# DIAGNijmegen/bodyct-dram-emph-subtype

Hardware: AMD Instinct MI355X
Metric: CT volumes/sec (train step, 1x128x256x256) (higher is better)
Workload: dtype f32; 1 GPU; BASELINE configs[1]: resnet18segcls train step (fwd+loss+bwd+Adam), batch 2/GPU, 1x128x256x256, fp32, inputs resident in HBM; global_batch=2, parallelism=dp1, hip_graph=False, streams=2

## Files before the change

### bodyct-dram-emph-subtype_amd/csrc/stem.hip

```cpp
#include "common.h"

namespace {

constexpr int PZ = 13, PY = 21, PX = 21;
constexpr int PATCH = PZ * PY * PX;
constexpr int PXP = 24;
constexpr int PATCHP = PZ * PY * PXP;
constexpr int WLP = 96;
constexpr int KT = 50;
constexpr int WPT = (KT * 64 + 255) / 256;

struct StemGeom {
  int B, D, H, W, Do, Ho, Wo;
  int nz, ny, nx, tiles_per_b, nblk;
};

template <typename T>
__global__ __launch_bounds__(256, 2) void stem_fwd_kernel(const float* __restrict__ x,
                                                          const float* __restrict__ w,
                                                          T* __restrict__ y, float* __restrict__ stats,
                                                          const StemGeom g) {
  __shared__ __attribute__((aligned(16))) float lds[PATCHP + KT * WLP];
  float* patch = lds;
  float* wl = lds + PATCHP;
  const int tid = threadIdx.x, lane = tid & 63, wave = tid >> 6;
  const int li = lane & 31, lh = lane >> 5;

  int L = xcd_remap(blockIdx.x, g.nblk);
  const int b = L / g.tiles_per_b;
  int r = L - b * g.tiles_per_b;
  const int txi = r % g.nx; r /= g.nx;
  const int tyi = r % g.ny;
  const int tzi = r / g.ny;
  const int z0 = tzi * 4, y0 = tyi * 8, x0 = txi * 8;

  for (int idx = tid; idx < PATCH; idx += 256) {
    const int pz = idx / (PY * PX);
    const int rem = idx - pz * (PY * PX);
    const int py = rem / PX, px = rem - py * PX;
    const int zi = 2 * z0 - 3 + pz, yi = 2 * y0 - 3 + py, xi = 2 * x0 - 3 + px;
    const bool ok = (zi >= 0) & (zi < g.D) & (yi >= 0) & (yi < g.H) & (xi >= 0) & (xi < g.W);
    patch[(pz * PY + py) * PXP + px] = ok ? x[(((long)b * g.D + zi) * g.H + yi) * g.W + xi] : 0.f;
  }

  float rw[WPT];
  auto load_w = [&](int kz) {
#pragma unroll
    for (int p = 0; p < WPT; ++p) {
      const int idx = p * 256 + tid;
      const int t = idx >> 6, co = idx & 63;
      rw[p] = (idx < KT * 64 && t < 49) ? w[co * 343 + kz * 49 + t] : 0.f;
    }
  };
  auto store_w = [&]() {
#pragma unroll
    for (int p = 0; p < WPT; ++p) {
      const int idx = p * 256 + tid;
      if (idx < KT * 64) wl[(idx >> 6) * WLP + (idx & 63)] = rw[p];
    }
  };

  f32x16 acc[2][2];
#pragma unroll
  for (int mi = 0; mi < 2; ++mi)
#pragma unroll
    for (int nj = 0; nj < 2; ++nj)
#pragma unroll
      for (int e = 0; e < 16; ++e) acc[mi][nj][e] = 0.f;

  int abase[2];
#pragma unroll
  for (int mi = 0; mi < 2; ++mi) abase[mi] = (2 * wave) * (PY * PXP) + (2 * (4 * mi + (li >> 3))) * PXP + 2 * (li & 7);

  load_w(0);
  for (int kz = 0; kz < 7; ++kz) {
    __syncthreads();
    store_w();
    __syncthreads();
    if (kz + 1 < 7) load_w(kz + 1);
    const float* pk = patch + kz * (PY * PXP);
#pragma unroll
    for (int kk = 0; kk < KT / 2; ++kk) {
      constexpr int dummy = 0;
      (void)dummy;
      const int k0 = 2 * kk, k1 = 2 * kk + 1;
      const int o0 = (k0 < 49) ? (k0 / 7) * PXP + (k0 % 7) : 0;
      const int o1 = (k1 < 49) ? (k1 / 7) * PXP + (k1 % 7) : 0;
      const int ko = lh ? o1 : o0;
      const float a0 = pk[abase[0] + ko];
      const float a1 = pk[abase[1] + ko];
      const float b0 = wl[(2 * kk + lh) * WLP + li];
      const float b1 = wl[(2 * kk + lh) * WLP + 32 + li];
      acc[0][0] = __builtin_amdgcn_mfma_f32_32x32x2f32(a0, b0, acc[0][0], 0, 0, 0);
      acc[0][1] = __builtin_amdgcn_mfma_f32_32x32x2f32(a0, b1, acc[0][1], 0, 0, 0);
      acc[1][0] = __builtin_amdgcn_mfma_f32_32x32x2f32(a1, b0, acc[1][0], 0, 0, 0);
      acc[1][1] = __builtin_amdgcn_mfma_f32_32x32x2f32(a1, b1, acc[1][1], 0, 0, 0);
    }
  }

  float s1[2] = {0.f, 0.f}, s2[2] = {0.f, 0.f};
#pragma unroll
  for (int mi = 0; mi < 2; ++mi) {
#pragma unroll
    for (int e = 0; e < 16; ++e) {
      const int row = wave * 64 + mi * 32 + (e & 3) + 8 * (e >> 2) + 4 * lh;
      const int zo = z0 + (row >> 6), yo = y0 + ((row >> 3) & 7), xo = x0 + (row & 7);
      if ((zo < g.Do) & (yo < g.Ho) & (xo < g.Wo)) {
        const long o = ((((long)b * g.Do + zo) * g.Ho + yo) * g.Wo + xo) * 64 + li;
#pragma unroll
        for (int nj = 0; nj < 2; ++nj) {
          const float v = acc[mi][nj][e];
          st1<T>(y, o + nj * 32, v);
          s1[nj] += v;
          s2[nj] += v * v;
        }
      }
    }
  }
  if (stats) {
    __syncthreads();
    float* red = lds;
#pragma unroll
    for (int nj = 0; nj < 2; ++nj) {
      const float t1 = s1[nj] + __shfl_xor(s1[nj], 32, 64);
      const float t2 = s2[nj] + __shfl_xor(s2[nj], 32, 64);
      if (lh == 0) {
        red[(wave * 2 + 0) * 64 + nj * 32 + li] = t1;
        red[(wave * 2 + 1) * 64 + nj * 32 + li] = t2;
      }
    }
    __syncthreads();
    if (tid < 128) {
      const int which = tid >> 6, c = tid & 63;
      const float v = red[(0 + which) * 64 + c] + red[(2 + which) * 64 + c] + red[(4 + which) * 64 + c] +
                      red[(6 + which) * 64 + c];
      stats[((long)L * 2 + which) * 64 + c] = v;
    }
  }
}

constexpr int GZ = 7, GY = 21, GX = 21;
constexpr int GPATCH = GZ * GY * GX;
constexpr int GXP = 27;
constexpr int GPATCHP = GZ * GY * GXP;
constexpr int NTAP = 352;
constexpr int GLDY = 96;
constexpr int GPT = (GPATCH + 255) / 256;

struct StemWGeom {
  int B, D, H, W, Do, Ho, Wo;
  int ny, nx;
  int total;
};

template <typename T>
__global__ __launch_bounds__(256, 2) void stem_wgrad_kernel(const float* __restrict__ x,
                                                            const T* __restrict__ dy,
                                                            float* __restrict__ slab, const StemWGeom g) {
  __shared__ __attribute__((aligned(16))) float lds[GPATCHP + 3 + 64 * GLDY];
  float* patch = lds;
  float* dyl = lds + GPATCHP + 3;
  const int tid = threadIdx.x, lane = tid & 63, wave = tid >> 6;
  const int li = lane & 31, lh = lane >> 5;
  const int ntw = (wave < 3) ? 3 : 2;

  int toff[3];
#pragma unroll
  for (int j = 0; j < 3; ++j) {
    const int tap = 32 * (wave + 4 * j) + li;
    const int kz = tap / 49, rem = tap - kz * 49, ky = rem / 7, kx = rem - ky * 7;
    toff[j] = (tap < 343 ? kz * (GY * GXP) + ky * GXP + kx : 0) + 2 * lh;
  }

  f32x16 acc[3][2];
#pragma unroll
  for (int j = 0; j < 3; ++j)
#pragma unroll
    for (int mi = 0; mi < 2; ++mi)
#pragma unroll
      for (int e = 0; e < 16; ++e) acc[j][mi][e] = 0.f;

  float rp[GPT];
  float4 rd[4];
  auto load_tile = [&](int st) {
    int r = st;
    const int txi = r % g.nx; r /= g.nx;
    const int tyi = r % g.ny; r /= g.ny;
    const int zo = r % g.Do;
    const int b = r / g.Do;
    const int y0 = tyi * 8, x0 = txi * 8;
#pragma unroll
    for (int p = 0; p < GPT; ++p) {
      const int idx = p * 256 + tid;
      const int pz = idx / (GY * GX);
      const int rem = idx - pz * (GY * GX);
      const int py = rem / GX, px = rem - py * GX;
      const int zi = 2 * zo - 3 + pz, yi = 2 * y0 - 3 + py, xi = 2 * x0 - 3 + px;
      const bool ok = (idx < GPATCH) & (zi >= 0) & (zi < g.D) & (yi >= 0) & (yi < g.H) & (xi >= 0) & (xi < g.W);
      rp[p] = ok ? x[(((long)b * g.D + zi) * g.H + yi) * g.W + xi] : 0.f;
    }
#pragma unroll
    for (int p = 0; p < 4; ++p) {
      const int idx = p * 256 + tid;
      const int v = idx >> 4, c4 = idx & 15;
      const int yo = y0 + (v >> 3), xo = x0 + (v & 7);
      const bool ok = (yo < g.Ho) & (xo < g.Wo);
      const long o = ((((long)b * g.Do + zo) * g.Ho + yo) * g.Wo + xo) * 64 + c4 * 4;
      rd[p] = ok ? ld4<T>(dy, o) : make_float4(0.f, 0.f, 0.f, 0.f);
    }
  };
  auto store_tile = [&]() {
#pragma unroll
    for (int p = 0; p < GPT; ++p) {
      const int idx = p * 256 + tid;
      if (idx < GPATCH) {
        const int pz = idx / (GY * GX), rem = idx - pz * (GY * GX);
        patch[(pz * GY + rem / GX) * GXP + rem % GX] = rp[p];
      }
    }
#pragma unroll
    for (int p = 0; p < 4; ++p) {
      const int idx = p * 256 + tid;
      *reinterpret_cast<float4*>(&dyl[(idx >> 4) * GLDY + (idx & 15) * 4]) = rd[p];
    }
  };

  int st = blockIdx.x;
  if (st < g.total) load_tile(st);
  for (; st < g.total; st += gridDim.x) {
    __syncthreads();
    store_tile();
    __syncthreads();
    if (st + (int)gridDim.x < g.total) load_tile(st + gridDim.x);
#pragma unroll 8
    for (int kk = 0; kk < 32; ++kk) {
      const int vbase = (2 * (kk >> 2)) * GXP + 4 * (kk & 3);
      const float a0 = dyl[(2 * kk + lh) * GLDY + li];
      const float a1 = dyl[(2 * kk + lh) * GLDY + 32 + li];
#pragma unroll
      for (int j = 0; j < 3; ++j) {
        if (j < ntw) {
          const float bv = patch[vbase + toff[j]];
          acc[j][0] = __builtin_amdgcn_mfma_f32_32x32x2f32(a0, bv, acc[j][0], 0, 0, 0);
          acc[j][1] = __builtin_amdgcn_mfma_f32_32x32x2f32(a1, bv, acc[j][1], 0, 0, 0);
        }
      }
    }
  }
  float* sl = slab + (long)blockIdx.x * 64 * NTAP;
#pragma unroll
  for (int j = 0; j < 3; ++j) {
    if (j < ntw) {
#pragma unroll
      for (int mi = 0; mi < 2; ++mi)
#pragma unroll
        for (int e = 0; e < 16; ++e) {
          const int co = 32 * mi + (e & 3) + 8 * (e >> 2) + 4 * lh;
          sl[co * NTAP + 32 * (wave + 4 * j) + li] = acc[j][mi][e];
        }
    }
  }
}

__global__ __launch_bounds__(256) void stem_wgrad_reduce_kernel(const float* __restrict__ slab, float* __restrict__ dw,
                                                                int nslab) {
  __shared__ float part[4][64];
  const int r = threadIdx.x & 63, kg = threadIdx.x >> 6;
  const int i = blockIdx.x * 64 + r;
  const bool live = i < 64 * NTAP;
  float p[8];
// ... 9 lines not shown
  }
  part[kg][r] = ((p[0] + p[1]) + (p[2] + p[3])) + ((p[4] + p[5]) + (p[6] + p[7]));
  __syncthreads();
  if (kg == 0 && live) {
    const int co = i / NTAP, tap = i - co * NTAP;
    if (tap < 343) dw[co * 343 + tap] = (part[0][r] + part[1][r]) + (part[2][r] + part[3][r]);
  }
}

inline int stem_out(int n) { return (n + 6 - 7) / 2 + 1; }
inline int stem_wgrad_blocks(int total) { return total < 512 ? total : 512; }

}

extern "C" int dram_stem_num_tiles(int B, int Do, int Ho, int Wo) {
  return B * ((Do + 3) / 4) * ((Ho + 7) / 8) * ((Wo + 7) / 8);
}

template <typename T>
static int stem_fwd_impl(const float* x, const float* w, T* y, float* stats_partial, int B, int D, int H, int W,
                         dram_stream_t stream) {
  if (!x || !w || !y || B < 1 || D < 1 || H < 1 || W < 1) return DRAM_ERR_BAD_ARG;
  StemGeom g{};
  g.B = B; g.D = D; g.H = H; g.W = W;
  g.Do = stem_out(D); g.Ho = stem_out(H); g.Wo = stem_out(W);
  if ((long long)B * g.Do * g.Ho * g.Wo * 64 >= (1LL << 31)) return DRAM_ERR_UNSUPPORTED;
  g.nz = (g.Do + 3) / 4; g.ny = (g.Ho + 7) / 8; g.nx = (g.Wo + 7) / 8;
  g.tiles_per_b = g.nz * g.ny * g.nx;
  g.nblk = B * g.tiles_per_b;
  const double vo = (double)B * g.Do * g.Ho * g.Wo;
  DramProf prof(DRAM_FAM_STEM, 0, 2.0 * vo * 64.0 * 343.0,
                4.0 * ((double)B * D * H * W + 64.0 * 343.0) + sizeof(T) * vo * 64.0, (hipStream_t)stream);
  hipLaunchKernelGGL((stem_fwd_kernel<T>), dim3(g.nblk), dim3(256), 0, (hipStream_t)stream, x, w, y, stats_partial, g);
  DRAM_LAUNCH_CHECK();
  return DRAM_OK;
}
extern "C" int dram_stem_fwd(const float* x, const float* w, float* y, float* stats_partial, int B, int D,
                             int H, int W, dram_stream_t stream) {
  return stem_fwd_impl<float>(x, w, y, stats_partial, B, D, H, W, stream);
}
extern "C" int dram_stem_fwd_bf16(const float* x, const float* w, void* y, float* stats_partial, int B, int D,
                                  int H, int W, dram_stream_t stream) {
  return stem_fwd_impl<bf16_t>(x, w, (bf16_t*)y, stats_partial, B, D, H, W, stream);
}

extern "C" size_t dram_stem_bwd_weight_workspace(int B, int D, int H, int W) {
  const int Do = stem_out(D), Ho = stem_out(H), Wo = stem_out(W);
  const int total = B * Do * ((Ho + 7) / 8) * ((Wo + 7) / 8);
  return (size_t)stem_wgrad_blocks(total) * 64 * NTAP * sizeof(float);
}

template <typename T>
static int stem_bwd_weight_impl(const float* x, const T* dy, float* dw, int B, int D, int H, int W, void* workspace,
                                size_t workspace_bytes, dram_stream_t stream) {
  if (!x || !dy || !dw || B < 1 || D < 1 || H < 1 || W < 1) return DRAM_ERR_BAD_ARG;
  StemWGeom g{};
  g.B = B; g.D = D; g.H = H; g.W = W;
  g.Do = stem_out(D); g.Ho = stem_out(H); g.Wo = stem_out(W);
  g.ny = (g.Ho + 7) / 8; g.nx = (g.Wo + 7) / 8;
  g.total = B * g.Do * g.ny * g.nx;
  const int nblk = stem_wgrad_blocks(g.total);
  if (!workspace || workspace_bytes < (size_t)nblk * 64 * NTAP * sizeof(float)) return DRAM_ERR_WORKSPACE;
  hipStream_t s = (hipStream_t)stream;
  const double vo = (double)B * g.Do * g.Ho * g.Wo;
  DramProf prof(DRAM_FAM_STEM, 1, 2.0 * vo * 64.0 * 343.0,
                4.0 * ((double)B * D * H * W + 64.0 * 343.0) + sizeof(T) * vo * 64.0, s);
  hipLaunchKernelGGL((stem_wgrad_kernel<T>), dim3(nblk), dim3(256), 0, s, x, dy, (float*)workspace, g);
  DRAM_LAUNCH_CHECK();
  hipLaunchKernelGGL(stem_wgrad_reduce_kernel, dim3((64 * NTAP + 63) / 64), dim3(256), 0, s,
                     (const float*)workspace, dw, nblk);
  DRAM_LAUNCH_CHECK();
  return DRAM_OK;
}
extern "C" int dram_stem_bwd_weight(const float* x, const float* dy, float* dw, int B, int D, int H, int W,
                                    void* workspace, size_t workspace_bytes, dram_stream_t stream) {
  return stem_bwd_weight_impl<float>(x, dy, dw, B, D, H, W, workspace, workspace_bytes, stream);
}
extern "C" int dram_stem_bwd_weight_bf16(const float* x, const void* dy, float* dw, int B, int D, int H, int W,
                                         void* workspace, size_t workspace_bytes, dram_stream_t stream) {
  return stem_bwd_weight_impl<bf16_t>(x, (const bf16_t*)dy, dw, B, D, H, W, workspace, workspace_bytes, stream);
}
```

### bodyct-dram-emph-subtype_amd/engine.py

```python
from __future__ import annotations

import os
import time
from typing import Dict, List, Optional

import torch

from . import ops
from .ops import ConvGeom

Tensor = torch.Tensor

ARCHS = {
    "resnet18": ("basic", (2, 2, 2, 2)),
    "resnet34": ("basic", (3, 4, 6, 3)),
    "resnet50": ("bottleneck", (3, 4, 6, 3)),
}
EXPANSION = {"basic": 1, "bottleneck": 4}
STAGES = ((64, 1, 1), (128, 2, 1), (256, 1, 2), (512, 1, 4))
BN_EPS = 1e-5
BN_MOMENTUM = 0.1


class _State:
# ... 36 lines not shown

    def _bn_fwd(self, st: _State, y: Tensor, sp: Optional[Tensor], bnp: str, residual, rs, relu=True, pool=False,
                apply=True):
        P = st.P
        count = float(y.numel() // y.shape[-1])
        count_dev = None
        if st.training:
            if st.dist is not None and st.dist.sync_bn:
                flat, sums = ops.reduce_partials(sp, tail=count)
                st.dist.all_reduce_stats(flat)
                count_dev = flat[-1:]
                mean, invstd, scale, shift = ops.bn_finalize(sums, count, P[bnp + ".weight"], P[bnp + ".bias"],
                                                             P[bnp + ".running_mean"], P[bnp + ".running_var"],
                                                             BN_MOMENTUM, BN_EPS, True, count_dev)
            else:
                mean, invstd, scale, shift = ops.bn_fold_finalize(sp, count, P[bnp + ".weight"], P[bnp + ".bias"],
                                                                  P[bnp + ".running_mean"], P[bnp + ".running_var"],
                                                                  BN_MOMENTUM, BN_EPS)
            st.nbt.append(P[bnp + ".num_batches_tracked"])
        else:
            mean, invstd, scale, shift = ops.bn_finalize(None, 1.0, P[bnp + ".weight"], P[bnp + ".bias"],
                                                         P[bnp + ".running_mean"], P[bnp + ".running_var"],
                                                         BN_MOMENTUM, BN_EPS, False)
            if st.need_grad:
                st.eval_ss[bnp] = (scale, shift)
        if not apply:
            z = None
        elif pool:
            z = ops.bn_maxpool_fwd(y, scale, shift)
        else:
            z = ops.bn_apply(y, scale, shift, residual, rs, relu)
        return z, mean, invstd, (count, count_dev), (None if residual is not None else (scale, shift))

    def _bn_bwd_eval(self, st: _State, c: dict, dz: Tensor) -> Tensor:
        bnp = c["bn"]
        scale, shift = st.eval_ss[bnp]
        zmask = c["z"] if c.get("ss") is None else None
        if st.dist is not None:
            self._flush_wgrad(st)
        if st.need_param:
            part = ops.bn_bwd_reduce(dz, zmask, c["y"], c["mean"], c["invstd"], True, scale, shift)
            _, sf = ops.reduce_partials(part, want_f32=True)
            st.grads[bnp + ".weight"] = sf[1]
            st.grads[bnp + ".bias"] = sf[0]
        y = c["y"] if zmask is None else None
        if c.get("b") and st.need_param:
            dy, colpart = ops.bn_bwd_apply_eval(dz, zmask, y, scale, shift, True, want_colsum=True)
            if colpart is None:
                colpart = ops.colsum(dy)
            st.grads[c["b"]] = ops.reduce_partials(colpart)[0].float()
            return dy
        return ops.bn_bwd_apply_eval(dz, zmask, y, scale, shift, True)

    def _bn_bwd(self, st: _State, c: dict, dz: Tensor) -> Tensor:
        if not st.training:
            return self._bn_bwd_eval(st, c, dz)
        bnp = c["bn"]
        zmask, (sc, sh) = (c["z"], (None, None)) if c.get("ss") is None else (None, c["ss"])
        part = c.pop("part", None)
        if part is None:
            part = ops.bn_bwd_reduce(dz, zmask, c["y"], c["mean"], c["invstd"], True, sc, sh)
        sums, sf = ops.reduce_partials(part, want_f32=True)
        st.grads[bnp + ".weight"] = sf[1]
        st.grads[bnp + ".bias"] = sf[0]
        count, count_dev = c["count"]
        if st.dist is not None and st.dist.sync_bn:
            work = st.dist.all_reduce_stats_async(sums)
            self._flush_wgrad(st)
            work.wait()
        if c.get("b"):
            dy, colpart = ops.bn_bwd_apply(dz, zmask, c["y"], c["mean"], c["invstd"], st.P[bnp + ".weight"], sums,
                                           count, True, sc, sh, want_colsum=True, count_dev=count_dev)
            if colpart is None:
                colpart = ops.colsum(dy)
            st.grads[c["b"]] = ops.reduce_partials(colpart)[0].float()
            return dy
        return ops.bn_bwd_apply(dz, zmask, c["y"], c["mean"], c["invstd"], st.P[bnp + ".weight"], sums, count,
                                True, sc, sh, count_dev=count_dev)

    def _conv_bn_fwd(self, st: _State, x, wname: str, bname: Optional[str], bnp: str, k: int, stride: int,
                     pad: int, dil: int, residual=None, rs: int = 1, xr=None, defer_z: bool = False):
        w = st.P[wname]
        pro = None
        split = None
        if isinstance(x, tuple):
            split = x
            x = None
            B, D, H, W, _ = split[0].shape
            Cin = split[0].shape[4] + split[1].shape[4]
        elif isinstance(x, dict):
            B, D, H, W, Cin = x["y"].shape
            g = ConvGeom(B, D, H, W, Cin, w.shape[0], k, stride, pad, dil, self.tol)
            if k == 3 and ops.conv_prologue_ok(g, x["y"].dtype):
                pro, x = x["ss"], x["y"]
            else:
                x = ops.bn_apply(x["y"], x["ss"][0], x["ss"][1], None, 1, True)
        if split is None:
            B, D, H, W, Cin = x.shape
        g = ConvGeom(B, D, H, W, Cin, w.shape[0], k, stride, pad, dil, self.tol)
        st.convs.append((wname, g))
        if st.need_grad:
            pre = st.packed.pop(wname, None)
            if pre is not None and pre[2] == g:
                if st.packed_ready is not None:
                    torch.cuda.current_stream().wait_event(st.packed_ready)
                    st.packed_ready = None
                wf, wb = pre[0], pre[1]
            else:
                wf, wb = ops.pack_conv_weight(w, True, True, g, st.storage)
        else:
            wf, wb = ops.packed_forward_weight(w, g, st.storage), None
        if split is not None:
            y, sp, v = ops.conv3d_fwd_cat(split[0], split[1], wf, st.P[bname] if bname else None, g, st.training,
                                          st.need_param and not st.recompute)
        else:
            y, sp, v = ops.conv3d_fwd_keep(x, wf, st.P[bname] if bname else None, g, st.training,
                                           st.need_param and not st.recompute, prologue=pro)
        defer_z = defer_z and residual is None
        z, mean, invstd, count, ss = self._bn_fwd(st, y, sp, bnp, residual, rs, apply=not defer_z)
        c = None
        if st.need_grad:
            if (pro is not None or split is not None) and xr is None:
# ... 351 lines not shown
            if g_outs[0] is not None:
                gpool[:, :n0] = g_outs[0] / denom[:, None]
            if g_outs[1] is not None:
                gpool[:, n0:] = g_outs[1] / denom[:, None]
        gd = None
        if g_dense[0] is not None or g_dense[1] is not None:
            gd = torch.zeros_like(dense)
            if g_dense[0] is not None:
                gd[:, :n0] = g_dense[0]
            if g_dense[1] is not None:
                gd[:, n0:] = g_dense[1]
        return gpool, gd

    def _backward(self, saved, g_dense, g_outs):
        st: _State = saved["st"]
        dist = st.dist if st.need_param else None
        if dist is not None:
            dist.begin_backward(saved["dense"].device)
        if st.need_param and self._two_streams():
            st.side = ops.side_stream(saved["dense"].device.index)

        n0, n1 = saved["n0"], saved["n1"]
        NO = n0 + n1
        dense = saved["dense"]
        sig = self.head == "reg"
        gpool, gd = self._head_cotangents(saved, g_dense, g_outs)
        dxup3, wpart = ops.head_bwd(saved["xup3"], saved["hw"], dense if sig else None, gd, gpool,
                                    saved["lungs4"] if sig else None, sig)
        if st.need_param:
            wg = ops.reduce_partials(wpart.reshape(wpart.shape[0], 1, NO * 33)).reshape(NO, 33).float()
            st.grads["fcs.0.weight"] = wg[:n0, :32].reshape(n0, 32, 1, 1, 1).contiguous()
            st.grads["fcs.0.bias"] = wg[:n0, 32].contiguous()
            st.grads["fcs.1.weight"] = wg[n0:, :32].reshape(n1, 32, 1, 1, 1).contiguous()
            st.grads["fcs.1.bias"] = wg[n0:, 32].contiguous()
        if dist is not None:
            dist.grads_ready(st.grads, ["fcs.0.weight", "fcs.0.bias", "fcs.1.weight", "fcs.1.bias"])

        dxup2 = self._conv_bn_bwd(st, saved["cu3"], dxup3, nxt=saved["cu2"][1])
        dxup1, dskip_stem = self._up_bwd(st, saved["cu2"], dxup2, skip_view=True)
        d, dskip_x1 = self._up_bwd(st, saved["cu1"], dxup1)

        blocks = saved["blocks"]
        idx = len(blocks)
        for li in (3, 2, 1, 0):
            nblk = self.layers[li]
            for bi in reversed(range(nblk)):
                idx -= 1
                extra = dskip_x1 if (li == 1 and bi == 0) else None
                d = self._block_bwd(st, blocks[idx], d, extra_add=extra)
        self._flush_wgrad(st)
        dxs = ops.maxpool_bwd(d, saved["amax"], saved["xs_shape"], dskip_stem)
        c0 = dict(z=saved["xs"], y=saved["y0"], mean=saved["mean0"], invstd=saved["invstd0"], count=saved["count0"],
                  bn="bn1", ss=saved["ss0"])
        dy0 = self._bn_bwd(st, c0, dxs)
        if st.need_param:
            st.grads["conv1.weight"] = ops.stem_bwd_weight(saved["x4"], dy0,
                                                           out=dist.grad_out("conv1.weight") if dist else None)
        if st.need_x:
            x4 = saved["x4"]
            saved["dx"] = ops.stem_bwd_data(dy0, st.P["conv1.weight"], x4.shape).reshape(x4.shape[0], 1, *x4.shape[1:])
        if st.side is not None:
            torch.cuda.current_stream().wait_stream(st.side)
        if dist is not None:
            dist.grads_ready(st.grads, ["conv1.weight", "bn1.weight", "bn1.bias"])
            dist.finish(st.grads)
        return st.grads


def forward_decisions(saved: dict) -> Dict[str, Tensor]:
    def mask(z):
        return (z > 0).permute(0, 4, 1, 2, 3).contiguous()

    out = {"bn1": mask(saved["xs"]), "maxpool": saved["amax"].permute(0, 4, 1, 2, 3).contiguous()}
    units = []
    for blk in saved["blocks"]:
        units.extend(blk[:-1])
    for cu in (saved["cu1"], saved["cu2"]):
        units.extend(cu[:2])
    units.append(saved["cu3"])
    for c in units:
        if c["z"] is not None:
            out[c["bn"]] = mask(c["z"])
        else:
            sc, sh = c["ss"]
            with ops.launch_scope(c["y"].device):
                out[c["bn"]] = mask(ops.bn_apply(c["y"], sc, sh, None, 1, True))
    return out
```

### bodyct-dram-emph-subtype_amd/ops.py

```python
from __future__ import annotations

import contextlib
import ctypes
import os
import threading
import weakref
from dataclasses import dataclass
from typing import Dict, List, Optional, Tuple

import torch

from . import _lib
from ._lib import DramConvDesc

Tensor = torch.Tensor


def _L():
    return _lib.load()


_TLS = threading.local()


# ... 698 lines not shown
                _chk(_L().dram_wino_conv3d_bwd_weight(_p(x), _p(v_cache), _p(dy), _p(dw), d, _p(ws),
                                                      nbytes, _stream()), f"dram_wino_conv3d_bwd_weight{g}")
            return dw
    nbytes = plan.ws_direct_wgrad
    if nbytes == 0:
        raise RuntimeError(f"dram_conv3d_bwd_weight: unsupported geometry {g}")
    ws = _workspace(nbytes, x.device)
    with _span("conv_wgrad_kernel+reduce", g.flops, f"wgrad {g}"):
        _chk(_L().dram_conv3d_bwd_weight(_p(x), _p(dy), _p(dw), d, _p(ws), nbytes, _stream()),
             f"dram_conv3d_bwd_weight{g}")
    return dw


def stem_out(n: int) -> int:
    return (n + 6 - 7) // 2 + 1


def stem_fwd(x: Tensor, w: Tensor, want_stats: bool, out_dtype=torch.float32):
    _req(x, "x")
    if x.dim() != 4:
        raise ValueError("stem_fwd: x must be [B,D,H,W]")
    _req(w, "w", shape=(64, 1, 7, 7, 7))
    B, D, H, W = x.shape
    Do, Ho, Wo = stem_out(D), stem_out(H), stem_out(W)
    if out_dtype not in (torch.float32, BF16):
        raise TypeError(f"stem_fwd: unsupported storage type {out_dtype}")
    y = torch.empty((B, Do, Ho, Wo, 64), device=x.device, dtype=out_dtype)
    stats = None
    if want_stats:
        nt = _L().dram_stem_num_tiles(B, Do, Ho, Wo)
        stats = torch.empty((nt, 2, 64), device=x.device, dtype=torch.float32)
    with _span("stem_fwd_kernel", 2.0 * B * Do * Ho * Wo * 64 * 343):
        sfx = "" if out_dtype != BF16 else ("_bf16mm" if tuning_env("DRAM_STEM_BF16", "1") != "0" else "_bf16")
        _chk(_fn("dram_stem_fwd", sfx)(_p(x), _p(w), _p(y), _p(stats), B, D, H, W, _stream()), "dram_stem_fwd" + sfx)
    return y, stats


def stem_bwd_weight(x: Tensor, dy: Tensor, out: Optional[Tensor] = None) -> Tensor:
    _req(x, "x")
    B, D, H, W = x.shape
    sfx = _act(dy, "dy", (B, stem_out(D), stem_out(H), stem_out(W), 64))
    nbytes = _L().dram_stem_bwd_weight_workspace(B, D, H, W)
    ws = torch.empty(((nbytes + 3) // 4,), device=x.device, dtype=torch.float32)
    dw = out if out is not None else torch.empty((64, 1, 7, 7, 7), device=x.device, dtype=torch.float32)
    _req(dw, "dw", shape=(64, 1, 7, 7, 7))
    with _span("stem_wgrad_kernel+reduce", 2.0 * dy.numel() * 343):
        if sfx and tuning_env("DRAM_STEM_BF16", "1") != "0":
            sfx = "_bf16mm"
        _chk(_fn("dram_stem_bwd_weight", sfx)(_p(x), _p(dy), _p(dw), B, D, H, W, _p(ws), nbytes, _stream()),
             "dram_stem_bwd_weight" + sfx)
    return dw


def stem_bwd_data(dy: Tensor, w: Tensor, in_shape) -> Tensor:
    B, D, H, W = (int(v) for v in in_shape)
    if min(B, D, H, W) < 1:
        raise ValueError(f"stem_bwd_data: bad input shape {tuple(in_shape)}")
    sfx = _act(dy, "dy", (B, stem_out(D), stem_out(H), stem_out(W), 64))
    _req(w, "w", shape=(64, 1, 7, 7, 7))
    nbytes = _L().dram_stem_bwd_data_workspace(B, D, H, W)
    ws = torch.empty(((nbytes + 3) // 4,), device=dy.device, dtype=torch.float32)
    dx = torch.empty((B, D, H, W), device=dy.device, dtype=torch.float32)
    with _span("stem_dgrad_kernel+fold", 2.0 * dy.numel() * 343):
        _chk(_fn("dram_stem_bwd_data", sfx)(_p(dy), _p(w), _p(dx), B, D, H, W, _p(ws), nbytes, _stream()),
             "dram_stem_bwd_data" + sfx)
    return dx


FOLD_TICKET_DOUBLES = _lib.DRAM_FOLD_TICKET_DOUBLES


def reduce_partials(partial: Tensor, tail: Optional[float] = None, want_f32: bool = False):
    _req(partial, "partial")
    Pn, R, C = partial.shape
    stages = _L().dram_fold_partials_stages(Pn)
    n = R * C + (1 if tail is not None else 0)
    buf = torch.empty((n + stages * R * C + (FOLD_TICKET_DOUBLES if stages > 1 else 0),), device=partial.device,
                      dtype=torch.float64)
    flat = buf[:n]
    f32 = [torch.empty((C,), device=partial.device, dtype=torch.float32) for _ in range(R)] if want_f32 else None
    if want_f32 and R > 2:
        raise ValueError("reduce_partials: the float copy supports at most two rows")
    _chk(_L().dram_fold_partials(_p(partial), _p(flat), _p(buf[n:]), _p(f32[0]) if f32 else None,
                                 _p(f32[1]) if (f32 and R == 2) else None, Pn, R, C,
                                 float(tail) if tail is not None else 0.0, int(tail is not None), _stream()),
         "dram_fold_partials")
    res = (flat, flat[:R * C].view(R, C)) if tail is not None else (flat.view(R, C),)
    if want_f32:
        res = res + (f32,)
    return res if len(res) > 1 else res[0]


def bn_fold_finalize(partial: Tensor, count: float, gamma: Tensor, beta: Tensor, running_mean: Tensor,
                     running_var: Tensor, momentum: float, eps: float):
    _req(partial, "partial")
    Pn, R, C = partial.shape
    if R != 2:
        raise ValueError("bn_fold_finalize: expected [P,2,C] partial sums")
    for t, nm in ((gamma, "gamma"), (beta, "beta"), (running_mean, "running_mean"), (running_var, "running_var")):
        _req(t, nm, shape=(C,))
    stages = _L().dram_fold_partials_stages(Pn)
    buf = torch.empty(((1 + stages) * 2 * C + (FOLD_TICKET_DOUBLES if stages > 1 else 0),), device=partial.device,
                      dtype=torch.float64)
    out = torch.empty((4, C), device=partial.device, dtype=torch.float32)
    _chk(_L().dram_bn_fold_finalize(_p(partial), _p(buf), _p(buf[2 * C:]), Pn, C, float(count), _p(gamma), _p(beta),
                                    _p(running_mean), _p(running_var), float(momentum), float(eps), 1, _p(out[0]),
# ... 520 lines not shown
```

### include/dram_hip.h

```cpp
#ifndef DRAM_HIP_H
#define DRAM_HIP_H

#include <stddef.h>
#include <stdint.h>

#ifdef __cplusplus
extern "C" {
#endif

typedef void* dram_stream_t;

#define DRAM_OK 0
#define DRAM_ERR_BAD_ARG (-1)
#define DRAM_ERR_UNSUPPORTED (-2)
#define DRAM_ERR_WORKSPACE (-3)

#define DRAM_ABI_VERSION 7
int dram_version(void);
const char* dram_build_info(void);
const char* dram_abi_hash(void);
unsigned long long dram_stream_capture_id(dram_stream_t stream);

enum {
  DRAM_FAM_CONV_WINO2D = 0,
// ... 69 lines not shown
int dram_wino_conv3d_fwd(const float* x, const float* uf, const float* bias, float* y,
                         float* stats_partial, float* v_keep, const DramConvDesc* desc, void* workspace,
                         size_t workspace_bytes, dram_stream_t stream);
int dram_wino_prologue_supported(const DramConvDesc* d);
int dram_wino_conv3d_fwd_cat(const float* x0, int C0, const float* x1, int C1, const float* uf, const float* bias, float* y,
                             float* stats_partial, float* v_keep, const DramConvDesc* desc, void* workspace,
                             size_t workspace_bytes, dram_stream_t stream);
int dram_wino_conv3d_fwd_bn(const float* x_pre, const float* pscale, const float* pshift, const float* uf, const float* bias,
                            float* y, float* stats_partial, float* v_keep, const DramConvDesc* d, void* workspace,
                            size_t workspace_bytes, dram_stream_t stream);
int dram_wino_conv3d_bwd_data(const float* dy, const float* ub, float* dx, const float* add,
                              const float* gate, const DramConvDesc* desc, void* workspace,
                              size_t workspace_bytes, dram_stream_t stream);
int dram_wino_num_stat_rows_bwd(const DramConvDesc* desc);
int dram_wino_conv3d_bwd_data_bn(const float* dy, const float* ub, float* dx, const float* bn_y, const float* bn_mean,
                                 const float* bn_invstd, const float* bn_scale, const float* bn_shift,
                                 float* stats_partial, const DramConvDesc* desc, void* workspace, size_t workspace_bytes,
                                 dram_stream_t stream);
int dram_wino_conv3d_bwd_weight(const float* x, const float* v_cache, const float* dy, float* dw,
                                const DramConvDesc* desc, void* workspace, size_t workspace_bytes,
                                dram_stream_t stream);

int dram_wino2d_applicable(const DramConvDesc* desc);
int dram_wino2d_num_stat_rows(const DramConvDesc* desc);
int dram_wino2d_pack_weight(const float* w, float* uf, float* ub, int Cout, int Cin, dram_stream_t stream);
int dram_wino2d_conv3d_fwd(const float* x, const float* uf, const float* bias, float* y,
                           float* stats_partial, const DramConvDesc* desc, dram_stream_t stream);
int dram_wino2d_conv3d_bwd_data(const float* dy, const float* ub, float* dx, const float* add,
                                const float* gate, const DramConvDesc* desc, dram_stream_t stream);

int dram_wgrad_w2d_applicable(const DramConvDesc* desc);
size_t dram_wgrad_w2d_workspace(const DramConvDesc* desc);
int dram_wgrad_w2d(const float* x, const float* dy, float* dw, const DramConvDesc* desc, void* workspace,
                   size_t workspace_bytes, dram_stream_t stream);

int dram_conv1x1_applicable(const DramConvDesc* desc);
int dram_conv1x1_num_stat_rows(const DramConvDesc* desc);
int dram_conv1x1_fwd(const float* x, const float* w2d, const float* bias, float* y, float* stats_partial,
                     const DramConvDesc* desc, dram_stream_t stream);
int dram_conv1x1_bwd_data(const float* dy, const float* wt, float* dx, const float* add, const float* gate,
                          const DramConvDesc* desc, dram_stream_t stream);
size_t dram_conv1x1_bwd_weight_workspace(const DramConvDesc* desc);
int dram_conv1x1_bwd_weight(const float* x, const float* dy, float* dw, const DramConvDesc* desc, void* workspace,
                            size_t workspace_bytes, dram_stream_t stream);

int dram_conv_algo(const DramConvDesc* desc);

int dram_stem_num_tiles(int B, int Do, int Ho, int Wo);
int dram_stem_fwd(const float* x, const float* w, float* y, float* stats_partial, int B, int D, int H,
                  int W, dram_stream_t stream);
size_t dram_stem_bwd_weight_workspace(int B, int D, int H, int W);
int dram_stem_bwd_weight(const float* x, const float* dy, float* dw, int B, int D, int H, int W,
                         void* workspace, size_t workspace_bytes, dram_stream_t stream);
size_t dram_stem_bwd_data_workspace(int B, int D, int H, int W);
int dram_stem_bwd_data(const float* dy, const float* w, float* dx, int B, int D, int H, int W, void* workspace,
                       size_t workspace_bytes, dram_stream_t stream);

int dram_reduce_partials_stages(int nparts);
#define DRAM_FOLD_TICKET_DOUBLES 256
int dram_fold_partials_stages(int nparts);
int dram_fold_partials(const float* partial, double* sums, double* scratch, float* sums_f32, float* f32_row1, int nparts,
                       int R, int C, double tail, int has_tail, dram_stream_t stream);
int dram_bn_fold_finalize(const float* partial, double* sums, double* scratch, int nparts, int C, double count,
                          const float* gamma, const float* beta, float* running_mean, float* running_var, float momentum,
                          float eps, int update_running, float* mean, float* invstd, float* scale, float* shift,
                          dram_stream_t stream);
int dram_reduce_partials(const float* partial, double* sums, double* scratch, int nparts, int R, int C,
                         double tail, int has_tail, dram_stream_t stream);

int dram_bn_finalize(const double* sums, double count, const double* count_dev, const float* gamma, const float* beta,
                     float* running_mean, float* running_var, float momentum, float eps,
                     int update_running, float* mean, float* invstd, float* scale, float* shift,
                     int C, dram_stream_t stream);

int dram_bn_apply(const float* y, const float* scale, const float* shift, const float* residual,
                  int Dr, int Hr, int Wr, int Cr, int rs, float* z, int B, int D, int H, int W, int C,
                  int relu, dram_stream_t stream);

int dram_colsum_nparts(long long rows, int C);
int dram_bn_bwd_reduce(const float* dz, const float* z, const float* y, const float* mean,
                       const float* invstd, const float* scale, const float* shift, float* partial,
                       long long rows, int C, int relu, dram_stream_t stream);
int dram_bn_bwd_apply_nparts(long long rows, int C);
int dram_bn_bwd_apply(const float* dz, const float* z, const float* y, const float* mean,
                      const float* invstd, const float* gamma, const float* scale, const float* shift,
                      const double* sums, double count, const double* count_dev, float* dy,
                      float* colsum_partial, long long rows, int C, int relu, dram_stream_t stream);
int dram_bn_bwd_apply_eval(const float* dz, const float* z, const float* y, const float* scale, const float* shift,
                           float* dy, float* colsum_partial, long long rows, int C, int relu, dram_stream_t stream);
int dram_colsum(const float* a, float* partial, long long rows, int C, dram_stream_t stream);

int dram_maxpool_fwd(const float* x, float* y, uint8_t* argmax, int B, int D, int H, int W, int C,
                     dram_stream_t stream);
int dram_bn_maxpool_fwd(const float* y, const float* scale, const float* shift, float* z, float* pooled, uint8_t* argmax,
                        int B, int D, int H, int W, int C, dram_stream_t stream);
int dram_maxpool_bwd(const float* dy, const uint8_t* argmax, const float* add, int add_stride, float* dx,
                     int B, int D, int H, int W, int C, dram_stream_t stream);

int dram_upcat_fwd(const float* src, const float* skip, float* cat, int B, int Ds, int Hs, int Ws, int Cu,
                   int Dk, int Hk, int Wk, int Ck, dram_stream_t stream);
int dram_upcat_bwd(const float* dcat, float* dsrc, float* dskip, int B, int Ds, int Hs, int Ws, int Cu,
                   int Dk, int Hk, int Wk, int Ck, dram_stream_t stream);

int dram_upmix_stat_rows(long long nvox);
int dram_upmix_axis_fwd(const void* in, int in_bf16, float* out, long long outer, int Ni, int m, int C,
                        dram_stream_t stream);
// ... 196 lines not shown
```

Before: 54.53 volumes/sec.

## Fuse stem BN backward apply into stem weight-gradient kernel

When training without needing the input gradient, the stem BN backward (ReLU mask plus normalization correction) is computed inside the stem wgrad kernel's tile load, so the intermediate dy0 tensor is never written and re-read. The per-channel BN constants are staged in LDS. Separately, the stem forward patch load now uses clamped, row-structured global loads held in registers and stored to LDS after the weight prefetch. In exchange, the fused kernel reads y as well as dz, uses more registers, and is limited to fp32.

```diff
diff --git a/bodyct-dram-emph-subtype_amd/csrc/stem.hip b/bodyct-dram-emph-subtype_amd/csrc/stem.hip
--- a/bodyct-dram-emph-subtype_amd/csrc/stem.hip
+++ b/bodyct-dram-emph-subtype_amd/csrc/stem.hip
@@ -9,6 +9,8 @@
 constexpr int WLP = 96;
 constexpr int KT = 50;
 constexpr int WPT = (KT * 64 + 255) / 256;
+constexpr int FROWS = 256 / PX;
+constexpr int FPT = (PZ * PY + FROWS - 1) / FROWS;
 
 struct StemGeom {
   int B, D, H, W, Do, Ho, Wo;
@@ -34,13 +36,18 @@
   const int tzi = r / g.ny;
   const int z0 = tzi * 4, y0 = tyi * 8, x0 = txi * 8;
 
-  for (int idx = tid; idx < PATCH; idx += 256) {
-    const int pz = idx / (PY * PX);
-    const int rem = idx - pz * (PY * PX);
-    const int py = rem / PX, px = rem - py * PX;
-    const int zi = 2 * z0 - 3 + pz, yi = 2 * y0 - 3 + py, xi = 2 * x0 - 3 + px;
-    const bool ok = (zi >= 0) & (zi < g.D) & (yi >= 0) & (yi < g.H) & (xi >= 0) & (xi < g.W);
-    patch[(pz * PY + py) * PXP + px] = ok ? x[(((long)b * g.D + zi) * g.H + yi) * g.W + xi] : 0.f;
+  float rx[FPT];
+  const float* xb = x + (long)b * g.D * g.H * g.W;
+  const int ppx = tid % PX, prs = tid / PX;
+  const int pxi = 2 * x0 - 3 + ppx;
+  const bool pokx = (pxi >= 0) & (pxi < g.W) & (prs < FROWS);
+  const int pxc = min(max(pxi, 0), g.W - 1);
+#pragma unroll
+  for (int p = 0; p < FPT; ++p) {
+    const int row = min(p * FROWS + prs, PZ * PY - 1);
+    const int pz = row / PY, py = row - pz * PY;
+    const int zi = min(max(2 * z0 - 3 + pz, 0), g.D - 1), yi = min(max(2 * y0 - 3 + py, 0), g.H - 1);
+    rx[p] = xb[((long)zi * g.H + yi) * g.W + pxc];
   }
 
   float rw[WPT];
@@ -73,6 +80,14 @@
   for (int mi = 0; mi < 2; ++mi) abase[mi] = (2 * wave) * (PY * PXP) + (2 * (4 * mi + (li >> 3))) * PXP + 2 * (li & 7);
 
   load_w(0);
+#pragma unroll
+  for (int p = 0; p < FPT; ++p) {
+    const int row = p * FROWS + prs;
+    const int pz = row / PY, py = row - pz * PY;
+    const int zi = 2 * z0 - 3 + pz, yi = 2 * y0 - 3 + py;
+    const bool ok = pokx & (zi >= 0) & (zi < g.D) & (yi >= 0) & (yi < g.H);
+    if ((prs < FROWS) & (row < PZ * PY)) patch[row * PXP + ppx] = ok ? rx[p] : 0.f;
+  }
   for (int kz = 0; kz < 7; ++kz) {
     __syncthreads();
     store_w();
@@ -153,17 +168,49 @@
   int total;
 };
 
-template <typename T>
+struct StemBnArgs {
+  const float *y, *mean, *invstd, *gamma, *scale, *shift;
+  const double* sums;
+  double inv_count;
+  const double* count_dev;
+};
+constexpr int BNK = 7;
+
+__device__ __forceinline__ float bn_bwd_elem(float dz, float y, float sc, float sh, float mu, float is, float gi, float mg,
+                                             float mgx) {
+#pragma clang fp contract(off)
+  const float m = __builtin_fmaf(y, sc, sh);
+  const float g = m > 0.f ? dz : 0.f;
+  const float xh = (y - mu) * is;
+  return gi * __builtin_fmaf(-xh, mgx, g - mg);
+}
+
+template <typename T, bool BN>
 __global__ __launch_bounds__(256, 2) void stem_wgrad_kernel(const float* __restrict__ x,
                                                             const T* __restrict__ dy,
-                                                            float* __restrict__ slab, const StemWGeom g) {
+                                                            float* __restrict__ slab, const StemWGeom g,
+                                                            const StemBnArgs bn) {
   __shared__ __attribute__((aligned(16))) float lds[GPATCHP + 3 + 64 * GLDY];
+  __shared__ float4 cst[BN ? BNK * 16 : 1];
   float* patch = lds;
   float* dyl = lds + GPATCHP + 3;
   const int tid = threadIdx.x, lane = tid & 63, wave = tid >> 6;
   const int li = lane & 31, lh = lane >> 5;
   const int ntw = (wave < 3) ? 3 : 2;
 
+  if (BN && tid < 64) {
+    const double inv_count = bn.count_dev ? 1.0 / *bn.count_dev : bn.inv_count;
+    float* cf = reinterpret_cast<float*>(cst);
+    const float is = bn.invstd[tid];
+    cf[(0 * 16) * 4 + tid] = bn.scale[tid];
+    cf[(1 * 16) * 4 + tid] = bn.shift[tid];
+    cf[(2 * 16) * 4 + tid] = bn.mean[tid];
+    cf[(3 * 16) * 4 + tid] = is;
+    cf[(4 * 16) * 4 + tid] = bn.gamma[tid] * is;
+    cf[(5 * 16) * 4 + tid] = (float)(bn.sums[tid] * inv_count);
+    cf[(6 * 16) * 4 + tid] = (float)(bn.sums[64 + tid] * inv_count);
+  }
+
   int toff[3];
 #pragma unroll
   for (int j = 0; j < 3; ++j) {
@@ -181,7 +228,8 @@
       for (int e = 0; e < 16; ++e) acc[j][mi][e] = 0.f;
 
   float rp[GPT];
-  float4 rd[4];
+  float4 rd[4], ry[BN ? 4 : 1];
+  int okm = 0;
   auto load_tile = [&](int st) {
     int r = st;
     const int txi = r % g.nx; r /= g.nx;
@@ -189,6 +237,7 @@
     const int zo = r % g.Do;
     const int b = r / g.Do;
     const int y0 = tyi * 8, x0 = txi * 8;
+    const float* xb = x + (long)b * g.D * g.H * g.W;
 #pragma unroll
     for (int p = 0; p < GPT; ++p) {
       const int idx = p * 256 + tid;
@@ -197,16 +246,29 @@
       const int py = rem / GX, px = rem - py * GX;
       const int zi = 2 * zo - 3 + pz, yi = 2 * y0 - 3 + py, xi = 2 * x0 - 3 + px;
       const bool ok = (idx < GPATCH) & (zi >= 0) & (zi < g.D) & (yi >= 0) & (yi < g.H) & (xi >= 0) & (xi < g.W);
-      rp[p] = ok ? x[(((long)b * g.D + zi) * g.H + yi) * g.W + xi] : 0.f;
-    }
+      if (BN) {
+        const int zc = min(max(zi, 0), g.D - 1), yc = min(max(yi, 0), g.H - 1), xc = min(max(xi, 0), g.W - 1);
+        const float v = xb[((long)zc * g.H + yc) * g.W + xc];
+        rp[p] = ok ? v : 0.f;
+      } else {
+        rp[p] = ok ? xb[((long)zi * g.H + yi) * g.W + xi] : 0.f;
+      }
+    }
+    okm = 0;
 #pragma unroll
     for (int p = 0; p < 4; ++p) {
       const int idx = p * 256 + tid;
       const int v = idx >> 4, c4 = idx & 15;
       const int yo = y0 + (v >> 3), xo = x0 + (v & 7);
       const bool ok = (yo < g.Ho) & (xo < g.Wo);
-      const long o = ((((long)b * g.Do + zo) * g.Ho + yo) * g.Wo + xo) * 64 + c4 * 4;
-      rd[p] = ok ? ld4<T>(dy, o) : make_float4(0.f, 0.f, 0.f, 0.f);
+      const long o = ((((long)b * g.Do + zo) * g.Ho + min(yo, g.Ho - 1)) * g.Wo + min(xo, g.Wo - 1)) * 64 + c4 * 4;
+      if (BN) {
+        rd[p] = ld4<T>(dy, o);
+        ry[p] = ld4<float>(bn.y, o);
+        okm |= (int)ok << p;
+      } else {
+        rd[p] = ok ? ld4<T>(dy, o) : make_float4(0.f, 0.f, 0.f, 0.f);
+      }
     }
   };
   auto store_tile = [&]() {
@@ -216,6 +278,20 @@
       if (idx < GPATCH) {
         const int pz = idx / (GY * GX), rem = idx - pz * (GY * GX);
         patch[(pz * GY + rem / GX) * GXP + rem % GX] = rp[p];
+      }
+    }
+    if (BN) {
+      const int c4 = tid & 15;
+      const float4 sc = cst[0 * 16 + c4], sh = cst[1 * 16 + c4], mu = cst[2 * 16 + c4], is = cst[3 * 16 + c4];
+      const float4 gi = cst[4 * 16 + c4], mg = cst[5 * 16 + c4], mgx = cst[6 * 16 + c4];
+#pragma unroll
+      for (int p = 0; p < 4; ++p) {
+        const bool ok = (okm >> p) & 1;
+        const float4 d = rd[p], yv = ry[p];
+        rd[p].x = ok ? bn_bwd_elem(d.x, yv.x, sc.x, sh.x, mu.x, is.x, gi.x, mg.x, mgx.x) : 0.f;
+        rd[p].y = ok ? bn_bwd_elem(d.y, yv.y, sc.y, sh.y, mu.y, is.y, gi.y, mg.y, mgx.y) : 0.f;
+        rd[p].z = ok ? bn_bwd_elem(d.z, yv.z, sc.z, sh.z, mu.z, is.z, gi.z, mg.z, mgx.z) : 0.f;
+        rd[p].w = ok ? bn_bwd_elem(d.w, yv.w, sc.w, sh.w, mu.w, is.w, gi.w, mg.w, mgx.w) : 0.f;
       }
     }
 #pragma unroll
@@ -331,7 +407,7 @@
 
 template <typename T>
 static int stem_bwd_weight_impl(const float* x, const T* dy, float* dw, int B, int D, int H, int W, void* workspace,
-                                size_t workspace_bytes, dram_stream_t stream) {
+                                size_t workspace_bytes, dram_stream_t stream, const StemBnArgs* bn = nullptr) {
   if (!x || !dy || !dw || B < 1 || D < 1 || H < 1 || W < 1) return DRAM_ERR_BAD_ARG;
   StemWGeom g{};
   g.B = B; g.D = D; g.H = H; g.W = W;
@@ -343,8 +419,12 @@
   hipStream_t s = (hipStream_t)stream;
   const double vo = (double)B * g.Do * g.Ho * g.Wo;
   DramProf prof(DRAM_FAM_STEM, 1, 2.0 * vo * 64.0 * 343.0,
-                4.0 * ((double)B * D * H * W + 64.0 * 343.0) + sizeof(T) * vo * 64.0, s);
-  hipLaunchKernelGGL((stem_wgrad_kernel<T>), dim3(nblk), dim3(256), 0, s, x, dy, (float*)workspace, g);
+                4.0 * ((double)B * D * H * W + 64.0 * 343.0) + sizeof(T) * vo * 64.0 * (bn ? 2.0 : 1.0), s);
+  if constexpr (sizeof(T) == 4) {
+    if (bn) hipLaunchKernelGGL((stem_wgrad_kernel<T, true>), dim3(nblk), dim3(256), 0, s, x, dy, (float*)workspace, g, *bn);
+  }
+  if (!bn) hipLaunchKernelGGL((stem_wgrad_kernel<T, false>), dim3(nblk), dim3(256), 0, s, x, dy, (float*)workspace, g,
+                              StemBnArgs{});
   DRAM_LAUNCH_CHECK();
   hipLaunchKernelGGL(stem_wgrad_reduce_kernel, dim3((64 * NTAP + 63) / 64), dim3(256), 0, s,
                      (const float*)workspace, dw, nblk);
@@ -355,6 +435,16 @@
                                     void* workspace, size_t workspace_bytes, dram_stream_t stream) {
   return stem_bwd_weight_impl<float>(x, dy, dw, B, D, H, W, workspace, workspace_bytes, stream);
 }
+extern "C" int dram_stem_bwd_weight_bn(const float* x, const float* dz, const float* y, const float* mean,
+                                       const float* invstd, const float* gamma, const float* scale, const float* shift,
+                                       const double* sums, double inv_count, const double* count_dev, float* dw, int B,
+                                       int D, int H, int W, void* workspace, size_t workspace_bytes,
+                                       dram_stream_t stream) {
+  if (!y || !mean || !invstd || !gamma || !scale || !shift || !sums || (!count_dev && !(inv_count > 0.0)))
+    return DRAM_ERR_BAD_ARG;
+  const StemBnArgs bn{y, mean, invstd, gamma, scale, shift, sums, count_dev ? 0.0 : inv_count, count_dev};
+  return stem_bwd_weight_impl<float>(x, dz, dw, B, D, H, W, workspace, workspace_bytes, stream, &bn);
+}
 extern "C" int dram_stem_bwd_weight_bf16(const float* x, const void* dy, float* dw, int B, int D, int H, int W,
                                          void* workspace, size_t workspace_bytes, dram_stream_t stream) {
   return stem_bwd_weight_impl<bf16_t>(x, (const bf16_t*)dy, dw, B, D, H, W, workspace, workspace_bytes, stream);
diff --git a/bodyct-dram-emph-subtype_amd/engine.py b/bodyct-dram-emph-subtype_amd/engine.py
--- a/bodyct-dram-emph-subtype_amd/engine.py
+++ b/bodyct-dram-emph-subtype_amd/engine.py
@@ -112,9 +112,7 @@
             return dy
         return ops.bn_bwd_apply_eval(dz, zmask, y, scale, shift, True)
 
-    def _bn_bwd(self, st: _State, c: dict, dz: Tensor) -> Tensor:
-        if not st.training:
-            return self._bn_bwd_eval(st, c, dz)
+    def _bn_bwd_sums(self, st: _State, c: dict, dz: Tensor):
         bnp = c["bn"]
         zmask, (sc, sh) = (c["z"], (None, None)) if c.get("ss") is None else (None, c["ss"])
         part = c.pop("part", None)
@@ -123,11 +121,18 @@
         sums, sf = ops.reduce_partials(part, want_f32=True)
         st.grads[bnp + ".weight"] = sf[1]
         st.grads[bnp + ".bias"] = sf[0]
-        count, count_dev = c["count"]
         if st.dist is not None and st.dist.sync_bn:
             work = st.dist.all_reduce_stats_async(sums)
             self._flush_wgrad(st)
             work.wait()
+        return zmask, sc, sh, sums
+
+    def _bn_bwd(self, st: _State, c: dict, dz: Tensor) -> Tensor:
+        if not st.training:
+            return self._bn_bwd_eval(st, c, dz)
+        bnp = c["bn"]
+        zmask, sc, sh, sums = self._bn_bwd_sums(st, c, dz)
+        count, count_dev = c["count"]
         if c.get("b"):
             dy, colpart = ops.bn_bwd_apply(dz, zmask, c["y"], c["mean"], c["invstd"], st.P[bnp + ".weight"], sums,
                                            count, True, sc, sh, want_colsum=True, count_dev=count_dev)
@@ -585,10 +590,18 @@
         dxs = ops.maxpool_bwd(d, saved["amax"], saved["xs_shape"], dskip_stem)
         c0 = dict(z=saved["xs"], y=saved["y0"], mean=saved["mean0"], invstd=saved["invstd0"], count=saved["count0"],
                   bn="bn1", ss=saved["ss0"])
-        dy0 = self._bn_bwd(st, c0, dxs)
-        if st.need_param:
-            st.grads["conv1.weight"] = ops.stem_bwd_weight(saved["x4"], dy0,
-                                                           out=dist.grad_out("conv1.weight") if dist else None)
+        gw_out = dist.grad_out("conv1.weight") if (dist and st.need_param) else None
+        if st.training and st.need_param and not st.need_x and dxs.dtype == torch.float32:
+            _, sc, sh, sums = self._bn_bwd_sums(st, c0, dxs)
+            count, count_dev = c0["count"]
+            st.grads["conv1.weight"] = ops.stem_bwd_weight_bn(saved["x4"], dxs, c0["y"], c0["mean"], c0["invstd"],
+                                                              st.P["bn1.weight"], sc, sh, sums, count,
+                                                              count_dev=count_dev, out=gw_out)
+            dy0 = None
+        else:
+            dy0 = self._bn_bwd(st, c0, dxs)
+            if st.need_param:
+                st.grads["conv1.weight"] = ops.stem_bwd_weight(saved["x4"], dy0, out=gw_out)
         if st.need_x:
             x4 = saved["x4"]
             saved["dx"] = ops.stem_bwd_data(dy0, st.P["conv1.weight"], x4.shape).reshape(x4.shape[0], 1, *x4.shape[1:])
diff --git a/bodyct-dram-emph-subtype_amd/ops.py b/bodyct-dram-emph-subtype_amd/ops.py
--- a/bodyct-dram-emph-subtype_amd/ops.py
+++ b/bodyct-dram-emph-subtype_amd/ops.py
@@ -774,6 +774,30 @@
     return dw
 
 
+def stem_bwd_weight_bn(x: Tensor, dz: Tensor, y: Tensor, mean: Tensor, invstd: Tensor, gamma: Tensor, scale: Tensor,
+                       shift: Tensor, sums: Tensor, count: float, count_dev: Optional[Tensor] = None,
+                       out: Optional[Tensor] = None) -> Tensor:
+    _req(x, "x")
+    B, D, H, W = x.shape
+    shape = (B, stem_out(D), stem_out(H), stem_out(W), 64)
+    _req(y, "y", shape=shape)
+    _req(dz, "dz", shape=shape)
+    for t, nm in ((mean, "mean"), (invstd, "invstd"), (gamma, "gamma"), (scale, "scale"), (shift, "shift")):
+        _req(t, nm, shape=(64,))
+    _req(sums, "sums", dtype=torch.float64, shape=(2, 64))
+    if count_dev is not None:
+        _req(count_dev, "count_dev", dtype=torch.float64, shape=(1,))
+    nbytes = _L().dram_stem_bwd_weight_workspace(B, D, H, W)
+    ws = torch.empty(((nbytes + 3) // 4,), device=x.device, dtype=torch.float32)
+    dw = out if out is not None else torch.empty((64, 1, 7, 7, 7), device=x.device, dtype=torch.float32)
+    _req(dw, "dw", shape=(64, 1, 7, 7, 7))
+    with _span("stem_wgrad_kernel+reduce", 2.0 * dz.numel() * 343):
+        _chk(_L().dram_stem_bwd_weight_bn(_p(x), _p(dz), _p(y), _p(mean), _p(invstd), _p(gamma), _p(scale), _p(shift),
+                                          _p(sums), 1.0 / float(count), _p(count_dev), _p(dw), B, D, H, W, _p(ws),
+                                          nbytes, _stream()), "dram_stem_bwd_weight_bn")
+    return dw
+
+
 def stem_bwd_data(dy: Tensor, w: Tensor, in_shape) -> Tensor:
     B, D, H, W = (int(v) for v in in_shape)
     if min(B, D, H, W) < 1:
diff --git a/include/dram_hip.h b/include/dram_hip.h
--- a/include/dram_hip.h
+++ b/include/dram_hip.h
@@ -145,6 +145,10 @@
 size_t dram_stem_bwd_weight_workspace(int B, int D, int H, int W);
 int dram_stem_bwd_weight(const float* x, const float* dy, float* dw, int B, int D, int H, int W,
                          void* workspace, size_t workspace_bytes, dram_stream_t stream);
+int dram_stem_bwd_weight_bn(const float* x, const float* dz, const float* y, const float* mean, const float* invstd,
+                            const float* gamma, const float* scale, const float* shift, const double* sums,
+                            double inv_count, const double* count_dev, float* dw, int B, int D, int H, int W,
+                            void* workspace, size_t workspace_bytes, dram_stream_t stream);
 size_t dram_stem_bwd_data_workspace(int B, int D, int H, int W);
 int dram_stem_bwd_data(const float* dy, const float* w, float* dx, int B, int D, int H, int W, void* workspace,
                        size_t workspace_bytes, dram_stream_t stream);
```

Result: no change. 55.07 volumes/sec (median of 6 runs) (+1.0%).
